# VasylVaskivskyi/microaligner

Hardware: AMD Instinct MI355X
Metric: Mpix/s optical-flow reg+warp, 16k×16k float32 tile, 1/2/4/8 GPU (higher is better)
Workload: dtype f32

## Files before the change

### microaligner_amd/csrc/farneback.hip

```cpp
#include "ma_internal.h"

#include <algorithm>
#include <cmath>
#include <cfloat>
#include <type_traits>

namespace {

struct FbGeom {
    MaTiling t;
    int pitch;
    int tile0;
    size_t plane;
    int margin;
};

struct PolyConsts {
    float g0, g1, xg1, xxg1;
    double ig11, ig03, ig33, ig55;
};

enum { PL_R0 = 0, PL_R1 = 5, PL_M = 10, PL_V = 15, PL_COUNT = 20 };

__device__ __forceinline__ float* plane_ptr(float* ws, const FbGeom& g, int wl, int pl)
{
    return ws + ((size_t)wl * PL_COUNT + pl) * g.plane;
}

template <typename T>
__device__ __forceinline__ float fetch_window(const T* img, const MaTiling& t, int oy, int ox, int ly, int lx)
{
    int y = oy + ly, x = ox + lx;
    if ((unsigned)y < (unsigned)t.H && (unsigned)x < (unsigned)t.W) return (float)img[(size_t)y * t.W + x];
    return 0.f;
}

__device__ __forceinline__ void window_origin(const MaTiling& t, int widx, int& oy, int& ox)
{
    if (t.T == 0) { oy = 0; ox = 0; return; }
    int ty = widx / t.ntx, tx = widx - ty * t.ntx;
    oy = ty * t.T - t.ov;
    ox = tx * t.T - t.ov;
}

__device__ __forceinline__ void window_extent(const FbGeom& g, int oy, int ox, int& ey, int& ex)
{
    const int vy = min(g.t.Ph, g.t.H - oy), vx = min(g.t.Pw, g.t.W - ox);
    ey = min(g.t.Ph, vy + min(g.margin, g.t.Ph));
    ex = min(g.t.Pw, vx + min(g.margin, g.t.Pw));
}

struct FbRect { int y0, y1, x0, x1; };
__host__ __device__ __forceinline__ FbRect needed_rect_h(const MaTiling& t, int oy, int ox, int reach)
{
    FbRect r;
    if (t.T == 0) { r.y0 = 0; r.y1 = t.Ph; r.x0 = 0; r.x1 = t.Pw; return r; }
    const int cy1 = t.ov + t.T < t.H - oy ? t.ov + t.T : t.H - oy;
    const int cx1 = t.ov + t.T < t.W - ox ? t.ov + t.T : t.W - ox;
    r.y0 = t.ov - reach > 0 ? t.ov - reach : 0;
    r.x0 = t.ov - reach > 0 ? t.ov - reach : 0;
    r.y1 = cy1 + reach < t.Ph ? cy1 + reach : t.Ph;
    r.x1 = cx1 + reach < t.Pw ? cx1 + reach : t.Pw;
    return r;
}
__host__ __device__ __forceinline__ FbRect needed_rect_v(const MaTiling& t, int oy, int ox, int reach, int m)
{
    FbRect r = needed_rect_h(t, oy, ox, reach);
    r.x0 = r.x0 - m > 0 ? r.x0 - m : 0;
    r.x1 = r.x1 + m < t.Pw ? r.x1 + m : t.Pw;
    return r;
}
constexpr int NEED_XALIGN = 32;

constexpr int K1_TX = 64, K1_TY = 16, K1_THREADS = 256;

template <bool NEAR_BORDER = true>
__device__ __forceinline__ void update_matrices_px(const float r0[5], float r2, float r3, float r4, float r5,
                                                   float r6, bool inside, float dx, float dy, int x, int y,
                                                   int w, int h, float out[5])
{
    if (inside) {
        r4 = (r0[2] + r4) * 0.5f;
        r5 = (r0[3] + r5) * 0.5f;
        r6 = (r0[4] + r6) * 0.25f;
    } else {
        r2 = r3 = 0.f;
        r4 = r0[2];
        r5 = r0[3];
        r6 = r0[4] * 0.5f;
    }
    r2 = (r0[0] - r2) * 0.5f;
    r3 = (r0[1] - r3) * 0.5f;
    r2 += r4 * dy + r6 * dx;
    r3 += r6 * dy + r5 * dx;
    const int BORDER = 5;
    if (NEAR_BORDER && ((unsigned)(x - BORDER) >= (unsigned)(w - BORDER * 2) || (unsigned)(y - BORDER) >= (unsigned)(h - BORDER * 2))) {
        const float border[5] = {0.14f, 0.14f, 0.4472f, 0.4472f, 0.4472f};
        float scale = (x < BORDER ? border[x] : 1.f) * (x >= w - BORDER ? border[w - x - 1] : 1.f) *
                      (y < BORDER ? border[y] : 1.f) * (y >= h - BORDER ? border[h - y - 1] : 1.f);
        r2 *= scale; r3 *= scale; r4 *= scale; r5 *= scale; r6 *= scale;
    }
    out[0] = r4 * r4 + r6 * r6;
    out[1] = (r4 + r5) * r6;
    out[2] = r5 * r5 + r6 * r6;
    out[3] = r4 * r2 + r6 * r3;
    out[4] = r6 * r2 + r5 * r3;
}

template <typename T>
// ... 35 lines not shown
    for (int img = 0; img < 2; img++) {
        const T* src = img == 0 ? prev : next;
        if (sizeof(T) == 1 && interior) {
            constexpr int DW = RW / 4;
            const uint8_t* base = reinterpret_cast<const uint8_t*>(src) + (size_t)(oy + y0 - 2) * g.t.W + (ox + x0 - 2);
            for (int e = tid; e < RH * DW; e += K1_THREADS) {
                const int j = e / DW, dw = e - j * DW;
                uint32_t word;
                __builtin_memcpy(&word, base + (size_t)j * g.t.W + 4 * dw, 4);
                raw[j][4 * dw + 0] = (float)(word & 255u);
                raw[j][4 * dw + 1] = (float)((word >> 8) & 255u);
                raw[j][4 * dw + 2] = (float)((word >> 16) & 255u);
                raw[j][4 * dw + 3] = (float)(word >> 24);
            }
        } else {
            float v[RH / 4], vh = 0.f;
#pragma unroll
            for (int k = 0; k < RH / 4; k++)
                v[k] = fetch_window(src, g.t, oy, ox, d_reflect101(y0 - 2 + lyg + 4 * k, Ph), rtx0);
            if (hr4 < RH) vh = fetch_window(src, g.t, oy, ox, d_reflect101(y0 - 2 + hr4, Ph), rtxh);
#pragma unroll
            for (int k = 0; k < RH / 4; k++) raw[lyg + 4 * k][lx] = v[k];
            if (hr4 < RH) raw[hr4][hc4] = vh;
        }
        __syncthreads();
#pragma unroll
        for (int k = 0; k < RH / 4; k++) {
            const int j = lyg + 4 * k;
            tb[j][lx] = raw[j][tcx0] * 0.5f + (raw[j][tcx0 - 1] + raw[j][tcx0 + 1]) * 0.25f;
        }
        if (hr2 < RH) tb[hr2][hc2] = raw[hr2][tcxh] * 0.5f + (raw[hr2][tcxh - 1] + raw[hr2][tcxh + 1]) * 0.25f;
        __syncthreads();
#pragma unroll
        for (int k = 0; k < (K1_TY + 2 + 3) / 4; k++) {
            const int j = lyg + 4 * k;
            if (j < K1_TY + 2) {
                const int cy = d_clamp(d_clamp(y0 - 1 + j, 0, Ph - 1) - (y0 - 2), 1, RH - 2);
                bl[j][lx] = tb[cy][lx] * 0.5f + (tb[cy - 1][lx] + tb[cy + 1][lx]) * 0.25f;
            }
        }
        if (hr2 < K1_TY + 2) {
            const int cy = d_clamp(d_clamp(y0 - 1 + hr2, 0, Ph - 1) - (y0 - 2), 1, RH - 2);
            bl[hr2][hc2] = tb[cy][hc2] * 0.5f + (tb[cy - 1][hc2] + tb[cy + 1][hc2]) * 0.25f;
        }
        __syncthreads();
        auto vpass = [&](int j, int c) {
            float up = bl[j][c], ce = bl[j + 1][c], dn = bl[j + 2][c];
            float p = up + dn;
            float row0 = ce * pc.g0;
            vt[0][j][c] = row0 + pc.g1 * p;
            vt[1][j][c] = 0.f + pc.xg1 * (dn - up);
            vt[2][j][c] = 0.f + pc.xxg1 * p;
        };
#pragma unroll
        for (int k = 0; k < K1_TY / 4; k++) vpass(lyg + 4 * k, lx);
        if (hr2 < K1_TY) vpass(hr2, hc2);
        __syncthreads();
#pragma unroll
        for (int rr = 0; rr < 4; rr++) {
            __builtin_amdgcn_sched_barrier(0);
            const int j = lyg * 4 + rr;
            const int y = y0 + j, x = x0 + lx;
            const int c = lx + 1;
            float a0m = vt[0][j][c - 1], a0 = vt[0][j][c], a0p = vt[0][j][c + 1];
            float a1m = vt[1][j][c - 1], a1 = vt[1][j][c], a1p = vt[1][j][c + 1];
            float a2m = vt[2][j][c - 1], a2 = vt[2][j][c], a2p = vt[2][j][c + 1];
            double b1 = (double)(a0 * pc.g0), b3 = (double)(a1 * pc.g0), b5 = (double)(a2 * pc.g0);
            double tg = (double)(a0p + a0m);
            b1 += tg * (double)pc.g1;
            double b4 = 0.0 + tg * (double)pc.xxg1;
            double b2 = 0.0 + (double)((a0p - a0m) * pc.xg1);
            b3 += (double)((a1p + a1m) * pc.g1);
            double b6 = 0.0 + (double)((a1p - a1m) * pc.xg1);
            b5 += (double)((a2p + a2m) * pc.g1);
            float R[5];
            R[1] = (float)(b2 * pc.ig11);
            R[0] = (float)(b3 * pc.ig11);
            R[3] = (float)(b1 * pc.ig03 + b4 * pc.ig33);
            R[2] = (float)(b1 * pc.ig03 + b5 * pc.ig33);
            R[4] = (float)(b6 * pc.ig55);
            const bool ok = y < Ph && x < Pw;
            const int pix4 = (y * g.pitch + x) * 4;
            if (ok) {
#pragma unroll
                for (int k = 0; k < 5; k++)
                    __builtin_amdgcn_raw_buffer_store_b32(__float_as_uint(R[k]), wrsrc, pix4,
                                                          ((img == 0 ? PL_R0 : PL_R1) + k) * plane4, ST_NT);
            }
            if (img == 0) {
#pragma unroll
                for (int k = 0; k < 5; k++) r0v[rr][k] = R[k];
            } else if (ok) {
                const bool inside = x < Pw - 1 && y < Ph - 1;
                float Mv[5];
                update_matrices_px(r0v[rr], R[0], R[1], R[2], R[3], R[4], inside, 0.f, 0.f, x, y, Pw, Ph, Mv);
#pragma unroll
                for (int k = 0; k < 5; k++)
                    __builtin_amdgcn_raw_buffer_store_b32(__float_as_uint(Mv[k]), wrsrc, pix4, (PL_M + k) * plane4, ST_NT);
            }
        }
        __syncthreads();
    }
}

constexpr int BV_WAVES = 6, BH_WAVES = 4;
template <int R, int NW, bool FUSED>
__global__ __launch_bounds__(64 * NW, BV_WAVES) void fb_blur_v(FbGeom g, int m, const float* __restrict__ taps,
                                                     float* __restrict__ ws, int nplanes, int reach)
{
    extern __shared__ float lds[];
    const int lane = threadIdx.x & 63;
    const int w = __builtin_amdgcn_readfirstlane(threadIdx.x >> 6);
    const int Ph = g.t.Ph, Pw = g.t.Pw;
    const int nbx = (Pw + 63) / 64, nby = (Ph + NW * R - 1) / (NW * R);
    const int nslots = (int)(((nplanes + 7) / 8) * 8);
    const int item = d_xcd_work_item(blockIdx.x, nbx * nby * nslots);
    const int by = item % nby, bx = (item / nby) % nbx;
    const int bz = d_xcd_unit(item / (nby * nbx), nplanes);
    if (bz >= nplanes) return;
    const int wl = bz / 5, ch = bz - wl * 5;
    const float* src = plane_ptr(ws, g, wl, PL_M + ch);
    float* dst = plane_ptr(ws, g, wl, PL_V + ch);
    int oy, ox, ey, ex;
    window_origin(g.t, g.tile0 + wl, oy, ox);
    window_extent(g, oy, ox, ey, ex);
    const FbRect need = needed_rect_v(g.t, oy, ox, reach, m);
    const int x0 = (need.x0 & ~(NEED_XALIGN - 1)) + bx * 64, y0 = need.y0 + by * (NW * R);
    if (x0 >= min(ex, need.x1) || y0 >= min(ey, need.y1)) return;

    constexpr int G = 2;
    const int rows = NW * R + 2 * m + 2 * G;
    const int xc = min(x0 + lane, Pw - 1);
    const bool xin = xc < ex;
    {
        constexpr int SB = 42;
        const unsigned xo = (unsigned)xc * 4u;
        const __amdgpu_buffer_rsrc_t rsrc = __builtin_amdgcn_make_buffer_rsrc(const_cast<float*>(src), 0,
                                                                               (int)(g.plane * sizeof(float)), 0x00020000);
        for (int j0 = w; j0 < rows; j0 += NW * SB) {
            float v[SB];
#pragma unroll
            for (int k = 0; k < SB; k++) {
                const int y = d_clamp(y0 - m - G + j0 + NW * k, 0, Ph - 1);
                v[k] = __uint_as_float(__builtin_amdgcn_raw_buffer_load_b32(rsrc, (int)xo, min(y, ey - 1) * g.pitch * 4, 0));
                if (y >= ey || !xin) v[k] = 0.f;
            }
#pragma unroll
            for (int k = 0; k < SB; k++)
                if (j0 + NW * k < rows) lds[(j0 + NW * k) * 64 + lane] = v[k];
        }
    }
    __syncthreads();

    if (y0 + w * R >= min(ey, need.y1)) return;
    float acc[R];
    d_sym_fir_slide_pk<R, FUSED, true>(lds + lane, G + m + w * R, m, taps, acc);
    const int x = x0 + lane;
    const __amdgpu_buffer_rsrc_t drsrc = __builtin_amdgcn_make_buffer_rsrc(dst, 0, (int)(g.plane * sizeof(float)), 0x00020000);
    if (x >= need.x0 && x < need.x1) {
#pragma unroll
        for (int r = 0; r < R; r++) {
            const int y = y0 + w * R + r;
            if (y < need.y1) __builtin_amdgcn_raw_buffer_store_b32(__float_as_uint(acc[r]), drsrc, x * 4, y * g.pitch * 4, 0);
        }
    }
}

template <int R, int NW, bool FUSED>
__global__ __launch_bounds__(64 * NW, BV_WAVES) void fb_blur_v_stream(FbGeom g, int m, const float* __restrict__ taps,
                                                            float* __restrict__ ws, int nplanes, int reach)
// ... 136 lines not shown
        xo[q] = xi >= ex ? (int)0x80000000 : xi * 4;
    }
    auto issue = [&](int ch) {
#pragma unroll
        for (int k = 0; k < RW; k++) {
            const int soff = (PL_V + ch) * plane4 + min(y0 + w + NW * k, Ph - 1) * g.pitch * 4;
#pragma unroll
            for (int q = 0; q < Q; q++)
                v[k][q] = __uint_as_float(__builtin_amdgcn_raw_buffer_load_b32(wrsrc, xo[q], soff, 0));
        }
    };
    auto commit = [&]() {
#pragma unroll
        for (int q = 0; q < Q; q++) {
            if (lane + 64 * q < cols) {
#pragma unroll
                for (int k = 0; k < RW; k++) lds[(w + NW * k) * lp + lane + 64 * q] = v[k][q];
            }
        }
    };

    float hs[5][R];
    const bool wave_needed = x0 + w * R < xend;
    issue(0);
#pragma unroll
    for (int ch = 0; ch < 5; ch++) {
        commit();
        __syncthreads();
        float acc[R];
        if (wave_needed) {
            d_sym_fir_slide_pk<R, FUSED, false>(lds + row * lp + hcol, G + m + w * R, m, taps, acc);
        } else {
#pragma unroll
            for (int r = 0; r < R; r++) acc[r] = 0.f;
        }
#pragma unroll
        for (int r = 0; r < R; r++) hs[ch][r] = acc[r];
        if (ch < 4) issue(ch + 1);
        __syncthreads();
    }

    constexpr int TP = TXW + 1;
    ma_f2* tb = reinterpret_cast<ma_f2*>(lds);
    if (wave_needed) {
#pragma unroll
        for (int r = 0; r < R; r++) {
            const double g11 = hs[0][r], g12 = hs[1][r], g22 = hs[2][r], h1 = hs[3][r], h2 = hs[4][r];
            const double idet = 1. / (g11 * g22 - g12 * g12 + 1e-3);
            const float dx = (float)((g11 * h2 - g12 * h1) * idet);
            const float dy = (float)((g22 * h1 - g12 * h2) * idet);
            tb[row * TP + hcol + w * R + r] = (ma_f2){dx, dy};
        }
    }
    __syncthreads();

    if (LAST) {
        float* frow = flow_out + (size_t)(oy + y0) * g.t.W * 2;
        const long long fbytes = (long long)min(ROWS, yend - y0) * g.t.W * 8;
        const __amdgpu_buffer_rsrc_t frsrc = __builtin_amdgcn_make_buffer_rsrc(
            frow, 0, (int)(fbytes < 0x7fffffffLL ? fbytes : 0x7fffffffLL), 0x00020000);
        for (int p = tid; p < ROWS * TXW; p += NT) {
            const int rh = p / TXW, c = p - rh * TXW;
            const int y = y0 + rh, x = x0 + c;
            if (y < yend && x >= need.x0 && x < xend) {
                const ma_f2 f = tb[rh * TP + c];
                __builtin_amdgcn_raw_buffer_store_b64(__builtin_bit_cast(ma_u2, f), frsrc, (rh * g.t.W + ox + x) * 8, 0, 0);
            }
        }
    } else {
        auto epilogue = [&](auto near_border_tag) {
            constexpr bool NEAR_BORDER = decltype(near_border_tag)::value;
            constexpr int DR = NT / TXW, DC = NT % TXW;
            const int pitch4 = g.pitch * 4;
            int rh = tid / TXW, c = tid - rh * TXW;
            int pix4 = ((y0 + rh) * g.pitch + x0 + c) * 4;
            int tbi = rh * TP + c;
            for (int p = tid; p < ROWS * TXW; p += NT, rh += DR, c += DC, pix4 += DR * pitch4 + DC * 4, tbi += DR * TP + DC) {
                if (c >= TXW) { c -= TXW; rh += 1; pix4 += pitch4 - TXW * 4; tbi += TP - TXW; }
                const int y = y0 + rh, x = x0 + c;
                if (y < yend && x >= need.x0 && x < xend) {
                    const ma_f2 f = tb[tbi];
                    const float dx = f.x, dy = f.y;
                    float r0[5];
#pragma unroll
                    for (int k = 0; k < 5; k++)
                        r0[k] = __uint_as_float(__builtin_amdgcn_raw_buffer_load_b32(wrsrc, pix4, (PL_R0 + k) * plane4, 0));
                    float fx = (float)x + dx, fy = (float)y + dy;
                    int x1 = d_cvfloor(fx), y1 = d_cvfloor(fy);
                    fx -= (float)x1; fy -= (float)y1;
                    float r[5] = {0.f, 0.f, 0.f, 0.f, 0.f};
                    const bool inside = (unsigned)x1 < (unsigned)(Pw - 1) && (unsigned)y1 < (unsigned)(Ph - 1);
                    const bool r1zero = x1 + 1 >= ex || y1 + 1 >= ey;
                    if (inside && !r1zero) {
                        float a00 = (1.f - fx) * (1.f - fy), a01 = fx * (1.f - fy), a10 = (1.f - fx) * fy,
                              a11 = fx * fy;
                        const int q0 = (int)(__umul24((unsigned)y1, (unsigned)g.pitch) + (unsigned)x1) * 4, q1 = q0 + pitch4;
#pragma unroll
                        for (int k = 0; k < 5; k++) {
                            const int so = (PL_R1 + k) * plane4;
                            const float s00 = __uint_as_float(__builtin_amdgcn_raw_buffer_load_b32(wrsrc, q0, so, 0));
                            const float s01 = __uint_as_float(__builtin_amdgcn_raw_buffer_load_b32(wrsrc, q0 + 4, so, 0));
                            const float s10 = __uint_as_float(__builtin_amdgcn_raw_buffer_load_b32(wrsrc, q1, so, 0));
                            const float s11 = __uint_as_float(__builtin_amdgcn_raw_buffer_load_b32(wrsrc, q1 + 4, so, 0));
                            r[k] = a00 * s00 + a01 * s01 + a10 * s10 + a11 * s11;
                        }
                    }
                    float Mv[5];
                    update_matrices_px<NEAR_BORDER>(r0, r[0], r[1], r[2], r[3], r[4], inside, dx, dy, x, y, Pw, Ph, Mv);
#pragma unroll
                    for (int k = 0; k < 5; k++)
                        __builtin_amdgcn_raw_buffer_store_b32(__float_as_uint(Mv[k]), wrsrc, pix4, (PL_M + k) * plane4, 0);
                }
            }
        };
        const bool near_border = x0 < 5 || x0 + TXW > Pw - 5 || y0 < 5 || y0 + ROWS > Ph - 5;
        if (near_border) epilogue(std::true_type{});
        else epilogue(std::false_type{});
    }
}

template <bool FUSED>
__global__ void fb_blur_v_simple(FbGeom g, int m, const float* __restrict__ taps, float* __restrict__ ws)
{
    const int x = blockIdx.x * blockDim.x + threadIdx.x, y = blockIdx.y;
    const int wl = blockIdx.z / 5, ch = blockIdx.z - wl * 5;
    if (x >= g.t.Pw) return;
    const float* src = plane_ptr(ws, g, wl, PL_M + ch);
    float* dst = plane_ptr(ws, g, wl, PL_V + ch);
    float s = src[(size_t)y * g.pitch + x] * taps[0];
    for (int i = 1; i <= m; i++) {
        float dn = src[(size_t)min(y + i, g.t.Ph - 1) * g.pitch + x];
        float up = src[(size_t)max(y - i, 0) * g.pitch + x];
        s = d_muladd<FUSED>(dn + up, MA_TAP(taps, i), s);
    }
    dst[(size_t)y * g.pitch + x] = s;
}

template <bool FUSED>
__global__ void fb_blur_h_solve_simple(FbGeom g, int m, const float* __restrict__ taps, float* __restrict__ ws,
                                       int last, float* __restrict__ flow_out)
{
    const int x = blockIdx.x * blockDim.x + threadIdx.x, y = blockIdx.y;
    const int wl = blockIdx.z;
    const int Ph = g.t.Ph, Pw = g.t.Pw;
    if (x >= Pw) return;
    float hsum[5];
    for (int ch = 0; ch < 5; ch++) {
        const float* src = plane_ptr(ws, g, wl, PL_V + ch) + (size_t)y * g.pitch;
        float s = src[x] * taps[0];
        for (int i = 1; i <= m; i++) s = d_muladd<FUSED>(src[max(x - i, 0)] + src[min(x + i, Pw - 1)], MA_TAP(taps, i), s);
        hsum[ch] = s;
    }
    double g11 = hsum[0], g12 = hsum[1], g22 = hsum[2], h1 = hsum[3], h2 = hsum[4];
    double idet = 1. / (g11 * g22 - g12 * g12 + 1e-3);
    float dx = (float)((g11 * h2 - g12 * h1) * idet);
    float dy = (float)((g22 * h1 - g12 * h2) * idet);
    int oy, ox;
    window_origin(g.t, g.tile0 + wl, oy, ox);
    if (last) {
        bool keep = g.t.T == 0 || (y >= g.t.ov && y < g.t.ov + g.t.T && x >= g.t.ov && x < g.t.ov + g.t.T);
        int iy = oy + y, ix = ox + x;
        if (keep && iy < g.t.H && ix < g.t.W)
            reinterpret_cast<float2*>(flow_out)[(size_t)iy * g.t.W + ix] = make_float2(dx, dy);
        return;
    }
    const float* R0p = plane_ptr(ws, g, wl, PL_R0);
    const float* R1p = plane_ptr(ws, g, wl, PL_R1);
    float* Mp = plane_ptr(ws, g, wl, PL_M);
    const size_t pix = (size_t)y * g.pitch + x;
    float r0[5];
    for (int k = 0; k < 5; k++) r0[k] = R0p[k * g.plane + pix];
    float fx = (float)x + dx, fy = (float)y + dy;
    int x1 = d_cvfloor(fx), y1 = d_cvfloor(fy);
    fx -= (float)x1; fy -= (float)y1;
    float r[5] = {0.f, 0.f, 0.f, 0.f, 0.f};
    const bool inside = (unsigned)x1 < (unsigned)(Pw - 1) && (unsigned)y1 < (unsigned)(Ph - 1);
    if (inside) {
        float a00 = (1.f - fx) * (1.f - fy), a01 = fx * (1.f - fy), a10 = (1.f - fx) * fy, a11 = fx * fy;
        const float* q = R1p + (size_t)y1 * g.pitch + x1;
        for (int k = 0; k < 5; k++) {
            const float* qk = q + k * g.plane;
            r[k] = a00 * qk[0] + a01 * qk[1] + a10 * qk[g.pitch] + a11 * qk[g.pitch + 1];
        }
    }
    float Mv[5];
    update_matrices_px(r0, r[0], r[1], r[2], r[3], r[4], inside, dx, dy, x, y, Pw, Ph, Mv);
    for (int k = 0; k < 5; k++) Mp[k * g.plane + pix] = Mv[k];
}

__global__ void fb_copy_planes(FbGeom g, const float* __restrict__ ws, int pl, float* __restrict__ out)
{
    const int x = blockIdx.x * blockDim.x + threadIdx.x, y = blockIdx.y, k = blockIdx.z;
    if (x >= g.t.Pw) return;
    out[((size_t)k * g.t.Ph + y) * g.t.Pw + x] = ws[((size_t)pl + k) * g.plane + (size_t)y * g.pitch + x];
}

struct RsTap { int s0, s1; float a0, a1; bool tail; };
__device__ __forceinline__ RsTap rs_tap_x(int d, double scale, int ssz)
{
    RsTap t;
    float f = (float)((d + 0.5) * scale - 0.5);
    int s = d_cvfloor(f);
    f -= (float)s;
    if (s < 0) { s = 0; f = 0.f; }
    t.tail = s + 1 >= ssz;
    if (t.tail) { s = ssz - 1; f = 0.f; }
    t.s0 = s; t.s1 = min(s + 1, ssz - 1);
    t.a0 = 1.f - f; t.a1 = f;
    return t;
}
__device__ __forceinline__ RsTap rs_tap_y(int d, double scale, int ssz)
{
    RsTap t;
    float f = (float)((d + 0.5) * scale - 0.5);
    const int s = d_cvfloor(f);
    f -= (float)s;
    t.s0 = d_clamp(s, 0, ssz - 1); t.s1 = d_clamp(s + 1, 0, ssz - 1);
    t.a0 = 1.f - f; t.a1 = f;
    t.tail = false;
    return t;
}

constexpr int LV_THREADS = 256, LV_CHUNK = 2048;
template <typename T, bool FUSED>
__global__ __launch_bounds__(LV_THREADS) void fb_level_rows(const T* __restrict__ src, int H, int W, int wk, double scale_x,
                                                            const float* __restrict__ k, int ksize, float* __restrict__ tmp)
{
    __shared__ float seg[LV_CHUNK];
    const int ncol = 2 * wk, r = ksize / 2;
    const int c0 = blockIdx.x * LV_THREADS, c = c0 + threadIdx.x;
    auto col_of = [&](int cc) { const RsTap t = rs_tap_x(cc >> 1, scale_x, W); return (cc & 1) ? t.s1 : t.s0; };
    const int lo = col_of(c0) - r, hi = col_of(min(c0 + LV_THREADS, ncol) - 1) + r;
    const int sc = c < ncol ? col_of(c) - r : 0;
    for (int y = blockIdx.y; y < H; y += gridDim.y) {
        const T* row = src + (size_t)y * W;
        float acc = 0.f;
        for (int cs = lo; cs <= hi; cs += LV_CHUNK) {
            const int n = min(LV_CHUNK, hi + 1 - cs);
            for (int i = threadIdx.x; i < n; i += LV_THREADS) seg[i] = (float)row[d_reflect101(cs + i, W)];
            __syncthreads();
            if (c < ncol) {
                const int j1 = min(ksize, cs + n - sc);
                for (int j = max(0, cs - sc); j < j1; j++) {
                    const float v = seg[sc + j - cs];
                    acc = j == 0 ? __fmul_rn(k[0], v) : d_muladd<FUSED>(k[j], v, acc);
                }
            }
            __syncthreads();
        }
        if (c < ncol) tmp[(size_t)y * ncol + c] = acc;
    }
}

template <bool FUSED>
__global__ __launch_bounds__(256) void fb_level_cols(const float* __restrict__ tmp, int H, int W, int wk, int hk,
                                                     double scale_x, double scale_y, int area, const float* __restrict__ k,
                                                     int ksize, float* __restrict__ dst, int pitch)
{
    const int dx = blockIdx.x * 256 + threadIdx.x;
    if (dx >= wk) return;
    const int ncol = 2 * wk, r = ksize / 2;
    const float* col = tmp + 2 * dx;
    auto blur = [&](int y, int t) {
        float d = __fmul_rn(k[r], col[(size_t)y * ncol + t]);
        for (int j = 1; j <= r; j++)
            d = d_muladd<FUSED>(k[r + j], col[(size_t)d_reflect101(y + j, H) * ncol + t] + col[(size_t)d_reflect101(y - j, H) * ncol + t], d);
        return d;
    };
    const RsTap tx = rs_tap_x(dx, scale_x, W);
    for (int dy = blockIdx.y; dy < hk; dy += gridDim.y) {
        float out;
        if (area) {
            const float b00 = blur(2 * dy, 0), b01 = blur(2 * dy, 1), b10 = blur(2 * dy + 1, 0), b11 = blur(2 * dy + 1, 1);
            out = ((b00 + b01) + (b10 + b11)) * 0.25f;
        } else {
            const RsTap ty = rs_tap_y(dy, scale_y, H);
            auto hpass = [&](int y) { return tx.tail ? blur(y, 0) : blur(y, 0) * tx.a0 + blur(y, 1) * tx.a1; };
            const float h0 = hpass(ty.s0), h1 = hpass(ty.s1);
            out = d_muladd<FUSED>(h0, ty.a0, h1 * ty.a1);
        }
        dst[(size_t)dy * pitch + dx] = out;
    }
}

__global__ __launch_bounds__(256) void fb_polyexp_plain(FbGeom g, PolyConsts pc, float* __restrict__ ws)
{
    const int x = blockIdx.x * 256 + threadIdx.x, img = blockIdx.z;
    const int Ph = g.t.Ph, Pw = g.t.Pw;
    if (x >= Pw) return;
    const float* src = ws + (size_t)(PL_V + img) * g.plane;
    float* dst = ws + (size_t)(img == 0 ? PL_R0 : PL_R1) * g.plane;
    for (int y = blockIdx.y; y < Ph; y += gridDim.y) {
        const float* up = src + (size_t)max(y - 1, 0) * g.pitch;
        const float* ce = src + (size_t)y * g.pitch;
        const float* dn = src + (size_t)min(y + 1, Ph - 1) * g.pitch;
        float vt[3][3];
#pragma unroll
        for (int i = 0; i < 3; i++) {
            const int xx = d_clamp(x - 1 + i, 0, Pw - 1);
            const float u = up[xx], cc = ce[xx], d = dn[xx];
            const float p = u + d;
            const float row0 = cc * pc.g0;
            vt[0][i] = row0 + pc.g1 * p;
            vt[1][i] = 0.f + pc.xg1 * (d - u);
            vt[2][i] = 0.f + pc.xxg1 * p;
        }
        const float a0m = vt[0][0], a0 = vt[0][1], a0p = vt[0][2];
        const float a1m = vt[1][0], a1 = vt[1][1], a1p = vt[1][2];
        const float a2m = vt[2][0], a2 = vt[2][1], a2p = vt[2][2];
        double b1 = (double)(a0 * pc.g0), b3 = (double)(a1 * pc.g0), b5 = (double)(a2 * pc.g0);
        const double tg = (double)(a0p + a0m);
        b1 += tg * (double)pc.g1;
        const double b4 = 0.0 + tg * (double)pc.xxg1;
        const double b2 = 0.0 + (double)((a0p - a0m) * pc.xg1);
        b3 += (double)((a1p + a1m) * pc.g1);
        const double b6 = 0.0 + (double)((a1p - a1m) * pc.xg1);
        b5 += (double)((a2p + a2m) * pc.g1);
        const size_t pix = (size_t)y * g.pitch + x;
        dst[1 * g.plane + pix] = (float)(b2 * pc.ig11);
        dst[0 * g.plane + pix] = (float)(b3 * pc.ig11);
        dst[3 * g.plane + pix] = (float)(b1 * pc.ig03 + b4 * pc.ig33);
        dst[2 * g.plane + pix] = (float)(b1 * pc.ig03 + b5 * pc.ig33);
        dst[4 * g.plane + pix] = (float)(b6 * pc.ig55);
    }
}

template <bool FUSED>
__global__ __launch_bounds__(256) void fb_flow_resize(const float* __restrict__ src, int sw, int sh, double scale_x,
                                                      double scale_y, float* __restrict__ dst, int dw, int dh)
{
    const int dx = blockIdx.x * 256 + threadIdx.x;
    if (dx >= dw) return;
    const RsTap tx = rs_tap_x(dx, scale_x, sw);
    for (int dy = blockIdx.y; dy < dh; dy += gridDim.y) {
        const RsTap ty = rs_tap_y(dy, scale_y, sh);
        const float* r0 = src + (size_t)ty.s0 * sw * 2;
        const float* r1 = src + (size_t)ty.s1 * sw * 2;
#pragma unroll
        for (int c = 0; c < 2; c++) {
            const float h0 = tx.tail ? r0[tx.s0 * 2 + c] : r0[tx.s0 * 2 + c] * tx.a0 + r0[tx.s1 * 2 + c] * tx.a1;
            const float h1 = tx.tail ? r1[tx.s0 * 2 + c] : r1[tx.s0 * 2 + c] * tx.a0 + r1[tx.s1 * 2 + c] * tx.a1;
            const float v = d_muladd<FUSED>(h0, ty.a0, h1 * ty.a1);
            dst[((size_t)dy * dw + dx) * 2 + c] = v * 2.f + 0.f;
        }
    }
}

__global__ __launch_bounds__(256) void fb_update_matrices(FbGeom g, const float* __restrict__ flow, float* __restrict__ ws)
{
    const int x = blockIdx.x * 256 + threadIdx.x;
    const int Ph = g.t.Ph, Pw = g.t.Pw;
    if (x >= Pw) return;
    const float* R0p = ws + (size_t)PL_R0 * g.plane;
    const float* R1p = ws + (size_t)PL_R1 * g.plane;
    float* Mp = ws + (size_t)PL_M * g.plane;
    for (int y = blockIdx.y; y < Ph; y += gridDim.y) {
        const size_t pix = (size_t)y * g.pitch + x;
        const float dx = flow[((size_t)y * Pw + x) * 2], dy = flow[((size_t)y * Pw + x) * 2 + 1];
        float r0[5];
#pragma unroll
        for (int k = 0; k < 5; k++) r0[k] = R0p[k * g.plane + pix];
        float fx = (float)x + dx, fy = (float)y + dy;
        const int x1 = d_cvfloor(fx), y1 = d_cvfloor(fy);
        fx -= (float)x1; fy -= (float)y1;
        float r[5] = {0.f, 0.f, 0.f, 0.f, 0.f};
        const bool inside = (unsigned)x1 < (unsigned)(Pw - 1) && (unsigned)y1 < (unsigned)(Ph - 1);
        if (inside) {
            const float a00 = (1.f - fx) * (1.f - fy), a01 = fx * (1.f - fy), a10 = (1.f - fx) * fy, a11 = fx * fy;
            const float* q = R1p + (size_t)y1 * g.pitch + x1;
#pragma unroll
            for (int k = 0; k < 5; k++) {
                const float* qk = q + k * g.plane;
                r[k] = a00 * qk[0] + a01 * qk[1] + a10 * qk[g.pitch] + a11 * qk[g.pitch + 1];
            }
        }
        float Mv[5];
        update_matrices_px(r0, r[0], r[1], r[2], r[3], r[4], inside, dx, dy, x, y, Pw, Ph, Mv);
#pragma unroll
        for (int k = 0; k < 5; k++) Mp[k * g.plane + pix] = Mv[k];
    }
}


bool chol_inverse6(double* A, double* b)
{
    const int m = 6, n = 6;
    for (int i = 0; i < m; i++) {
        int j;
        for (j = 0; j < i; j++) {
            double s = A[i * m + j];
            for (int k = 0; k < j; k++) s -= A[i * m + k] * A[j * m + k];
            A[i * m + j] = s * A[j * m + j];
        }
        double s = A[i * m + i];
        for (int k = 0; k < j; k++) { double t = A[i * m + k]; s -= t * t; }
        if (s < DBL_EPSILON) return false;
        A[i * m + i] = 1. / std::sqrt(s);
    }
    for (int i = 0; i < m; i++)
        for (int j = 0; j < n; j++) {
            double s = b[i * n + j];
            for (int k = 0; k < i; k++) s -= A[i * m + k] * b[k * n + j];
            b[i * n + j] = s * A[i * m + i];
        }
    for (int i = m - 1; i >= 0; i--)
        for (int j = 0; j < n; j++) {
            double s = b[i * n + j];
            for (int k = m - 1; k > i; k--) s -= A[k * m + i] * b[k * n + j];
            b[i * n + j] = s * A[i * m + i];
        }
    return true;
}

bool make_poly_consts(double sigma, PolyConsts* pc)
{
    const int n = 1;
    float gb[3], xgb[3], xxgb[3];
    float *gk = gb + n, *xg = xgb + n, *xxg = xxgb + n;
    if (sigma < FLT_EPSILON) sigma = n * 0.3;
    double s = 0.;
    for (int x = -n; x <= n; x++) {
        gk[x] = (float)std::exp(-x * x / (2 * sigma * sigma));
        s += gk[x];
    }
    s = 1. / s;
    for (int x = -n; x <= n; x++) {
        gk[x] = (float)(gk[x] * s);
        xg[x] = (float)(x * gk[x]);
        xxg[x] = (float)(x * x * gk[x]);
    }
    double G[36] = {0}, I6[36] = {0};
    for (int y = -n; y <= n; y++)
        for (int x = -n; x <= n; x++) {
            G[0] += gk[y] * gk[x];
            G[7] += gk[y] * gk[x] * x * x;
            G[21] += gk[y] * gk[x] * x * x * x * x;
            G[35] += gk[y] * gk[x] * x * x * y * y;
        }
    G[14] = G[3] = G[4] = G[18] = G[24] = G[7];
    G[28] = G[21];
    G[22] = G[27] = G[35];
    for (int i = 0; i < 6; i++) I6[i * 6 + i] = 1.;
    if (!chol_inverse6(G, I6)) return false;
    pc->g0 = gk[0]; pc->g1 = gk[1]; pc->xg1 = xg[1]; pc->xxg1 = xxg[1];
    pc->ig11 = I6[7]; pc->ig03 = I6[3]; pc->ig33 = I6[21]; pc->ig55 = I6[35];
    return true;
}

void make_window_taps(int winsize, std::vector<float>& k)
{
    int m = winsize / 2;
    k.resize(m + 1);
    double sigma = m * 0.3, s = 1;
    k[0] = (float)s;
    for (int i = 1; i <= m; i++) {
        float t = (float)std::exp(-i * i / (2 * sigma * sigma));
        k[i] = t;
// ... 114 lines not shown
              const float* taps, int iters, float* flow_out)
{
    float* ws = (float*)ctx->ws;
    const FbPlan p = plan_batch(g, nwin, m, iters);
    {
        MaProfScope ps(ctx, MA_K_POLYEXP_M0, p.px);
        dim3 grid((g.t.Pw + K1_TX - 1) / K1_TX, (g.t.Ph + K1_TY - 1) / K1_TY, nwin);
        hipLaunchKernelGGL((fb_polyexp_m0<T>), grid, dim3(K1_THREADS), 0, ctx->stream, prev, next, g, pc, ws);
    }
    run_iterations<FUSED>(ctx, g, p, nwin, m, taps, iters, flow_out);
    MA_HIP(hipGetLastError());
    return MA_OK;
}

int get_taps(ma_ctx* ctx, int winsize, const float** out)
{
    std::vector<float> k;
    make_window_taps(winsize, k);
    std::vector<float> t = ma_layout_taps(k);
    return ma_const_table(ctx, ((uint64_t)1 << 56) | (uint64_t)winsize, t.data(), t.size(), out);
}

int check_window(int Ph, int Pw)
{
    const size_t bytes = ma_fb_window_bytes(Ph, Pw);
    if (bytes <= MA_FB_WINDOW_MAX_BYTES) return MA_OK;
    ma_set_error("invalid argument: Farneback window of %d x %d px too large: its 20 planes take %zu bytes, the 32-bit "
                 "plane addressing allows %zu (5178 x 5178 is the largest square window)", Ph, Pw, bytes,
                 MA_FB_WINDOW_MAX_BYTES);
    return MA_EINVAL;
}

int farneback_impl(ma_ctx* ctx, const void* prev, const void* next, int dtype, int H, int W, int tile, int overlap,
                   int winsize, int iterations, int poly_n, double poly_sigma, int flags, float* flow_out,
                   float* R0_out, float* R1_out, float* M0_out)
{
    MA_REQUIRE(ctx && prev && next && flow_out, "NULL argument");
    MA_REQUIRE(dtype == MA_U8 || dtype == MA_U16 || dtype == MA_F32, "dtype must be u8/u16/f32");
    MA_REQUIRE(H > 0 && W > 0, "image must be non-empty");
    MA_REQUIRE(tile >= 0 && overlap >= 0, "tile/overlap must be >= 0");
    MA_REQUIRE(winsize >= 1, "winsize must be >= 1");
    MA_REQUIRE(iterations >= 1, "iterations must be >= 1");
    MA_REQUIRE(poly_n == 1, "only poly_n == 1 is supported (the value microaligner passes)");
    const MaTiling t = ma_make_tiling(H, W, tile, overlap);
    MA_TRY(check_window(t.Ph, t.Pw));
    MA_HIP(hipSetDevice(ctx->device));

    PolyConsts pc;
    if (!make_poly_consts(poly_sigma, &pc)) { ma_set_error("polynomial-expansion Gram matrix is singular"); return MA_EINVAL; }
    const float* taps = nullptr;
    MA_TRY(get_taps(ctx, winsize, &taps));
    const int m = winsize / 2;

    FbGeom g;
    g.t = t;
    g.pitch = (int)ma_align_up((size_t)g.t.Pw, 64);
    g.plane = (size_t)g.t.Ph * g.pitch;
    g.margin = 1 << 28;
    const int nwin_total = g.t.ntx * g.t.nty;
    const size_t per_win = g.plane * PL_COUNT * sizeof(float);
    MA_REQUIRE(per_win <= ctx->ws_limit, "one window does not fit the workspace limit");
    int batch = (int)(ctx->ws_limit / per_win);
    if (batch > nwin_total) batch = nwin_total;
    if ((long long)batch * 5 > 65535) batch = 65535 / 5;
    MA_TRY(ma_ws_reserve(ctx, per_win * batch));
    const bool fused = (flags & MA_FB_MULADD_FUSED) != 0;

    for (int t0 = 0; t0 < nwin_total; t0 += batch) {
        int n = nwin_total - t0 < batch ? nwin_total - t0 : batch;
        g.tile0 = t0;
        int rc;
#define RUN(TYPE)                                                                                           \
    rc = fused ? run_batch<TYPE, true>(ctx, (const TYPE*)prev, (const TYPE*)next, g, n, pc, m, taps, iterations, flow_out) \
               : run_batch<TYPE, false>(ctx, (const TYPE*)prev, (const TYPE*)next, g, n, pc, m, taps, iterations, flow_out)
        if (dtype == MA_U8) { RUN(uint8_t); }
        else if (dtype == MA_U16) { RUN(uint16_t); }
        else { RUN(float); }
#undef RUN
        if (rc != MA_OK) return rc;
    }
    if (R0_out || R1_out || M0_out) {
        dim3 grid((g.t.Pw + 255) / 256, g.t.Ph, 5);
        float* ws = (float*)ctx->ws;
        if (R0_out) hipLaunchKernelGGL(fb_copy_planes, grid, dim3(256), 0, ctx->stream, g, ws, (int)PL_R0, R0_out);
        if (R1_out) hipLaunchKernelGGL(fb_copy_planes, grid, dim3(256), 0, ctx->stream, g, ws, (int)PL_R1, R1_out);
        if (M0_out) hipLaunchKernelGGL(fb_copy_planes, grid, dim3(256), 0, ctx->stream, g, ws, (int)PL_M, M0_out);
        MA_HIP(hipGetLastError());
    }
    return MA_OK;
}

struct FbLevel { int w, h, ksize; double sigma; };

std::vector<FbLevel> level_table(int H, int W, int levels)
{
    const double pyr_scale = 0.5;
    int k;
    double scale = 1;
    for (k = 0; k < levels; k++) {
        scale *= pyr_scale;
        if (W * scale < 32 || H * scale < 32) break;
    }
    std::vector<FbLevel> L(k + 1);
    for (int i = 0; i <= k; i++) {
        double s = 1;
        for (int j = 0; j < i; j++) s *= pyr_scale;
        const double sigma = (1. / s - 1) * 0.5;
        L[i].sigma = sigma;
        L[i].ksize = std::max((int)std::lrint(sigma * 5) | 1, 3);
        L[i].w = (int)std::lrint(W * s);
        L[i].h = (int)std::lrint(H * s);
    }
    return L;
}

FbGeom level_geom(const FbLevel& l)
{
    FbGeom g;
    g.t = ma_make_tiling(l.h, l.w, 0, 0);
    g.pitch = (int)ma_align_up((size_t)l.w, 64);
    g.plane = (size_t)l.h * g.pitch;
    g.tile0 = 0;
    g.margin = 1 << 28;
    return g;
}

double rs_scale(int dsz, int ssz) { return 1. / ((double)dsz / ssz); }

struct FbLevelWs { size_t flow_off, total; };
FbLevelWs level_workspace(const std::vector<FbLevel>& L, int H)
{
    FbLevelWs r{0, 0};
    for (size_t k = 0; k < L.size(); k++) {
        const FbGeom g = level_geom(L[k]);
        size_t need = g.plane * PL_COUNT;
        if (k > 0) need += (size_t)H * 2 * L[k].w;
        r.flow_off = std::max(r.flow_off, need);
    }
    r.total = r.flow_off + (L.size() > 1 ? (size_t)L[1].h * L[1].w * 2 : 0);
    return r;
}

template <typename T, bool FUSED>
int run_levels(ma_ctx* ctx, const T* prev, const T* next, int H, int W, const std::vector<FbLevel>& L, size_t flow_off,
               const PolyConsts& pc, int m, const float* taps, int iters, float* flow_out)
{
    float* ws = (float*)ctx->ws;
    float* flow_lv = ws + flow_off;
    const int top = (int)L.size() - 1;
    for (int k = top; k >= 0; k--) {
        const FbLevel& l = L[k];
        FbGeom g = level_geom(l);
        const FbPlan p = plan_batch(g, 1, m, iters);
        const double px = (double)l.w * l.h;
        const unsigned gy = (unsigned)std::min(l.h, MA_GRID_Y_MAX);
        if (k == 0) {
            MaProfScope ps(ctx, MA_K_POLYEXP_M0, p.px);
            dim3 grid((l.w + K1_TX - 1) / K1_TX, (l.h + K1_TY - 1) / K1_TY, 1);
            hipLaunchKernelGGL((fb_polyexp_m0<T>), grid, dim3(K1_THREADS), 0, ctx->stream, prev, next, g, pc, ws);
        } else {
            std::vector<float> kt;
            ma_gaussian_kernel(l.ksize, l.sigma, kt);
            const float* dk = nullptr;
            MA_TRY(ma_const_table(ctx, ((uint64_t)4 << 56) | (uint64_t)k, kt.data(), kt.size(), &dk));
            const int area = W == 2 * l.w && H == 2 * l.h;
            const double sx = rs_scale(l.w, W), sy = rs_scale(l.h, H);
            float* tmp = ws + g.plane * PL_COUNT;
            {
                MaProfScope ps(ctx, MA_K_FB_LEVEL_IMG, 2 * px);
// ... 106 lines not shown
```

Baseline: 3559.

## Interleave first four polynomial coefficient planes for vectorized 128-bit loads and stores

Changes the R0/R1 workspace layout so coefficients 0-3 are stored interleaved as float4 per pixel, with coefficient 4 kept in a separate plane. Writers use one 128-bit store plus one 32-bit store, and the bilinear sampling in the matrix-update paths uses b128/b64 loads in place of twenty scattered 32-bit loads. The goal is fewer memory transactions and better cache-line use in the gather-heavy warp step. The cost is 4x wider stride for the interleaved part, and every consumer, including the plane-copy debug output, must agree on the new layout.

```diff
diff --git a/microaligner_amd/csrc/farneback.hip b/microaligner_amd/csrc/farneback.hip
--- a/microaligner_amd/csrc/farneback.hip
+++ b/microaligner_amd/csrc/farneback.hip
@@ -21,10 +21,25 @@
 };
 
 enum { PL_R0 = 0, PL_R1 = 5, PL_M = 10, PL_V = 15, PL_COUNT = 20 };
+constexpr int R_C4 = 4;
+
+typedef unsigned ma_u4 __attribute__((ext_vector_type(4)));
 
 __device__ __forceinline__ float* plane_ptr(float* ws, const FbGeom& g, int wl, int pl)
 {
     return ws + ((size_t)wl * PL_COUNT + pl) * g.plane;
+}
+
+__device__ __forceinline__ void r_load(const float* __restrict__ r, const FbGeom& g, size_t pix, float v[5])
+{
+    const float4 a = reinterpret_cast<const float4*>(r)[pix];
+    v[0] = a.x; v[1] = a.y; v[2] = a.z; v[3] = a.w;
+    v[4] = r[R_C4 * g.plane + pix];
+}
+__device__ __forceinline__ void r_store(float* __restrict__ r, const FbGeom& g, size_t pix, const float v[5])
+{
+    reinterpret_cast<float4*>(r)[pix] = make_float4(v[0], v[1], v[2], v[3]);
+    r[R_C4 * g.plane + pix] = v[4];
 }
 
 template <typename T>
@@ -226,10 +241,10 @@
             const bool ok = y < Ph && x < Pw;
             const int pix4 = (y * g.pitch + x) * 4;
             if (ok) {
-#pragma unroll
-                for (int k = 0; k < 5; k++)
-                    __builtin_amdgcn_raw_buffer_store_b32(__float_as_uint(R[k]), wrsrc, pix4,
-                                                          ((img == 0 ? PL_R0 : PL_R1) + k) * plane4, ST_NT);
+                const int so = (img == 0 ? PL_R0 : PL_R1) * plane4;
+                const ma_u4 r03 = {__float_as_uint(R[0]), __float_as_uint(R[1]), __float_as_uint(R[2]), __float_as_uint(R[3])};
+                __builtin_amdgcn_raw_buffer_store_b128(r03, wrsrc, pix4 * 4, so, ST_NT);
+                __builtin_amdgcn_raw_buffer_store_b32(__float_as_uint(R[4]), wrsrc, pix4, so + R_C4 * plane4, ST_NT);
             }
             if (img == 0) {
 #pragma unroll
@@ -532,9 +547,12 @@
                     const ma_f2 f = tb[tbi];
                     const float dx = f.x, dy = f.y;
                     float r0[5];
-#pragma unroll
-                    for (int k = 0; k < 5; k++)
-                        r0[k] = __uint_as_float(__builtin_amdgcn_raw_buffer_load_b32(wrsrc, pix4, (PL_R0 + k) * plane4, 0));
+                    {
+                        const ma_u4 a = __builtin_amdgcn_raw_buffer_load_b128(wrsrc, pix4 * 4, PL_R0 * plane4, 0);
+                        r0[0] = __uint_as_float(a.x); r0[1] = __uint_as_float(a.y);
+                        r0[2] = __uint_as_float(a.z); r0[3] = __uint_as_float(a.w);
+                        r0[4] = __uint_as_float(__builtin_amdgcn_raw_buffer_load_b32(wrsrc, pix4, (PL_R0 + R_C4) * plane4, 0));
+                    }
                     float fx = (float)x + dx, fy = (float)y + dy;
                     int x1 = d_cvfloor(fx), y1 = d_cvfloor(fy);
                     fx -= (float)x1; fy -= (float)y1;
@@ -545,15 +563,19 @@
                         float a00 = (1.f - fx) * (1.f - fy), a01 = fx * (1.f - fy), a10 = (1.f - fx) * fy,
                               a11 = fx * fy;
                         const int q0 = (int)(__umul24((unsigned)y1, (unsigned)g.pitch) + (unsigned)x1) * 4, q1 = q0 + pitch4;
-#pragma unroll
-                        for (int k = 0; k < 5; k++) {
-                            const int so = (PL_R1 + k) * plane4;
-                            const float s00 = __uint_as_float(__builtin_amdgcn_raw_buffer_load_b32(wrsrc, q0, so, 0));
-                            const float s01 = __uint_as_float(__builtin_amdgcn_raw_buffer_load_b32(wrsrc, q0 + 4, so, 0));
-                            const float s10 = __uint_as_float(__builtin_amdgcn_raw_buffer_load_b32(wrsrc, q1, so, 0));
-                            const float s11 = __uint_as_float(__builtin_amdgcn_raw_buffer_load_b32(wrsrc, q1 + 4, so, 0));
-                            r[k] = a00 * s00 + a01 * s01 + a10 * s10 + a11 * s11;
-                        }
+                        const int so = PL_R1 * plane4, so4 = (PL_R1 + R_C4) * plane4;
+                        const ma_u4 t00 = __builtin_amdgcn_raw_buffer_load_b128(wrsrc, q0 * 4, so, 0);
+                        const ma_u4 t01 = __builtin_amdgcn_raw_buffer_load_b128(wrsrc, q0 * 4 + 16, so, 0);
+                        const ma_u4 t10 = __builtin_amdgcn_raw_buffer_load_b128(wrsrc, q1 * 4, so, 0);
+                        const ma_u4 t11 = __builtin_amdgcn_raw_buffer_load_b128(wrsrc, q1 * 4 + 16, so, 0);
+                        const ma_u2 c0 = __builtin_amdgcn_raw_buffer_load_b64(wrsrc, q0, so4, 0);
+                        const ma_u2 c1 = __builtin_amdgcn_raw_buffer_load_b64(wrsrc, q1, so4, 0);
+                        const float s00[5] = {__uint_as_float(t00.x), __uint_as_float(t00.y), __uint_as_float(t00.z), __uint_as_float(t00.w), __uint_as_float(c0.x)};
+                        const float s01[5] = {__uint_as_float(t01.x), __uint_as_float(t01.y), __uint_as_float(t01.z), __uint_as_float(t01.w), __uint_as_float(c0.y)};
+                        const float s10[5] = {__uint_as_float(t10.x), __uint_as_float(t10.y), __uint_as_float(t10.z), __uint_as_float(t10.w), __uint_as_float(c1.x)};
+                        const float s11[5] = {__uint_as_float(t11.x), __uint_as_float(t11.y), __uint_as_float(t11.z), __uint_as_float(t11.w), __uint_as_float(c1.y)};
+#pragma unroll
+                        for (int k = 0; k < 5; k++) r[k] = a00 * s00[k] + a01 * s01[k] + a10 * s10[k] + a11 * s11[k];
                     }
                     float Mv[5];
                     update_matrices_px<NEAR_BORDER>(r0, r[0], r[1], r[2], r[3], r[4], inside, dx, dy, x, y, Pw, Ph, Mv);
@@ -619,7 +641,7 @@
     float* Mp = plane_ptr(ws, g, wl, PL_M);
     const size_t pix = (size_t)y * g.pitch + x;
     float r0[5];
-    for (int k = 0; k < 5; k++) r0[k] = R0p[k * g.plane + pix];
+    r_load(R0p, g, pix, r0);
     float fx = (float)x + dx, fy = (float)y + dy;
     int x1 = d_cvfloor(fx), y1 = d_cvfloor(fy);
     fx -= (float)x1; fy -= (float)y1;
@@ -627,22 +649,27 @@
     const bool inside = (unsigned)x1 < (unsigned)(Pw - 1) && (unsigned)y1 < (unsigned)(Ph - 1);
     if (inside) {
         float a00 = (1.f - fx) * (1.f - fy), a01 = fx * (1.f - fy), a10 = (1.f - fx) * fy, a11 = fx * fy;
-        const float* q = R1p + (size_t)y1 * g.pitch + x1;
-        for (int k = 0; k < 5; k++) {
-            const float* qk = q + k * g.plane;
-            r[k] = a00 * qk[0] + a01 * qk[1] + a10 * qk[g.pitch] + a11 * qk[g.pitch + 1];
-        }
+        const size_t q = (size_t)y1 * g.pitch + x1;
+        float s00[5], s01[5], s10[5], s11[5];
+        r_load(R1p, g, q, s00);
+        r_load(R1p, g, q + 1, s01);
+        r_load(R1p, g, q + g.pitch, s10);
+        r_load(R1p, g, q + g.pitch + 1, s11);
+        for (int k = 0; k < 5; k++) r[k] = a00 * s00[k] + a01 * s01[k] + a10 * s10[k] + a11 * s11[k];
     }
     float Mv[5];
     update_matrices_px(r0, r[0], r[1], r[2], r[3], r[4], inside, dx, dy, x, y, Pw, Ph, Mv);
     for (int k = 0; k < 5; k++) Mp[k * g.plane + pix] = Mv[k];
 }
 
-__global__ void fb_copy_planes(FbGeom g, const float* __restrict__ ws, int pl, float* __restrict__ out)
+__global__ void fb_copy_planes(FbGeom g, const float* __restrict__ ws, int pl, int interleaved, float* __restrict__ out)
 {
     const int x = blockIdx.x * blockDim.x + threadIdx.x, y = blockIdx.y, k = blockIdx.z;
     if (x >= g.t.Pw) return;
-    out[((size_t)k * g.t.Ph + y) * g.t.Pw + x] = ws[((size_t)pl + k) * g.plane + (size_t)y * g.pitch + x];
+    const size_t pix = (size_t)y * g.pitch + x;
+    const float* src = ws + (size_t)pl * g.plane;
+    out[((size_t)k * g.t.Ph + y) * g.t.Pw + x] = !interleaved ? src[k * g.plane + pix]
+                                                 : k < R_C4 ? src[pix * 4 + k] : src[R_C4 * g.plane + pix];
 }
 
 struct RsTap { int s0, s1; float a0, a1; bool tail; };
@@ -766,12 +793,13 @@
         b3 += (double)((a1p + a1m) * pc.g1);
         const double b6 = 0.0 + (double)((a1p - a1m) * pc.xg1);
         b5 += (double)((a2p + a2m) * pc.g1);
-        const size_t pix = (size_t)y * g.pitch + x;
-        dst[1 * g.plane + pix] = (float)(b2 * pc.ig11);
-        dst[0 * g.plane + pix] = (float)(b3 * pc.ig11);
-        dst[3 * g.plane + pix] = (float)(b1 * pc.ig03 + b4 * pc.ig33);
-        dst[2 * g.plane + pix] = (float)(b1 * pc.ig03 + b5 * pc.ig33);
-        dst[4 * g.plane + pix] = (float)(b6 * pc.ig55);
+        float R[5];
+        R[1] = (float)(b2 * pc.ig11);
+        R[0] = (float)(b3 * pc.ig11);
+        R[3] = (float)(b1 * pc.ig03 + b4 * pc.ig33);
+        R[2] = (float)(b1 * pc.ig03 + b5 * pc.ig33);
+        R[4] = (float)(b6 * pc.ig55);
+        r_store(dst, g, (size_t)y * g.pitch + x, R);
     }
 }
 
@@ -808,8 +836,7 @@
         const size_t pix = (size_t)y * g.pitch + x;
         const float dx = flow[((size_t)y * Pw + x) * 2], dy = flow[((size_t)y * Pw + x) * 2 + 1];
         float r0[5];
-#pragma unroll
-        for (int k = 0; k < 5; k++) r0[k] = R0p[k * g.plane + pix];
+        r_load(R0p, g, pix, r0);
         float fx = (float)x + dx, fy = (float)y + dy;
         const int x1 = d_cvfloor(fx), y1 = d_cvfloor(fy);
         fx -= (float)x1; fy -= (float)y1;
@@ -817,12 +844,14 @@
         const bool inside = (unsigned)x1 < (unsigned)(Pw - 1) && (unsigned)y1 < (unsigned)(Ph - 1);
         if (inside) {
             const float a00 = (1.f - fx) * (1.f - fy), a01 = fx * (1.f - fy), a10 = (1.f - fx) * fy, a11 = fx * fy;
-            const float* q = R1p + (size_t)y1 * g.pitch + x1;
-#pragma unroll
-            for (int k = 0; k < 5; k++) {
-                const float* qk = q + k * g.plane;
-                r[k] = a00 * qk[0] + a01 * qk[1] + a10 * qk[g.pitch] + a11 * qk[g.pitch + 1];
-            }
+            const size_t q = (size_t)y1 * g.pitch + x1;
+            float s00[5], s01[5], s10[5], s11[5];
+            r_load(R1p, g, q, s00);
+            r_load(R1p, g, q + 1, s01);
+            r_load(R1p, g, q + g.pitch, s10);
+            r_load(R1p, g, q + g.pitch + 1, s11);
+#pragma unroll
+            for (int k = 0; k < 5; k++) r[k] = a00 * s00[k] + a01 * s01[k] + a10 * s10[k] + a11 * s11[k];
         }
         float Mv[5];
         update_matrices_px(r0, r[0], r[1], r[2], r[3], r[4], inside, dx, dy, x, y, Pw, Ph, Mv);
@@ -1103,9 +1132,9 @@
     if (R0_out || R1_out || M0_out) {
         dim3 grid((g.t.Pw + 255) / 256, g.t.Ph, 5);
         float* ws = (float*)ctx->ws;
-        if (R0_out) hipLaunchKernelGGL(fb_copy_planes, grid, dim3(256), 0, ctx->stream, g, ws, (int)PL_R0, R0_out);
-        if (R1_out) hipLaunchKernelGGL(fb_copy_planes, grid, dim3(256), 0, ctx->stream, g, ws, (int)PL_R1, R1_out);
-        if (M0_out) hipLaunchKernelGGL(fb_copy_planes, grid, dim3(256), 0, ctx->stream, g, ws, (int)PL_M, M0_out);
+        if (R0_out) hipLaunchKernelGGL(fb_copy_planes, grid, dim3(256), 0, ctx->stream, g, ws, (int)PL_R0, 1, R0_out);
+        if (R1_out) hipLaunchKernelGGL(fb_copy_planes, grid, dim3(256), 0, ctx->stream, g, ws, (int)PL_R1, 1, R1_out);
+        if (M0_out) hipLaunchKernelGGL(fb_copy_planes, grid, dim3(256), 0, ctx->stream, g, ws, (int)PL_M, 0, M0_out);
         MA_HIP(hipGetLastError());
     }
     return MA_OK;
```

Result: no change. 3580 (median of 6 runs) (+0.6%).
